# satoken/dafs

Hardware: AMD Instinct MI355X
Metric: seq-pairs/sec (all-pairs ProbCons pair-HMM posteriors + sparse rows + sim) (higher is better)
Workload: dtype f32; 1 GPU; N=128 L~150 synthetic random RNA (seed 12345), 8128 pairs; align_model=ProbCons, kernel=k_pairhmm3<G=32,W=6> x 4064 waves

## Files before the change

dafs_amd/csrc/call_host.h:

```cpp
#pragma once
#include <errno.h>
#include <math.h>
#include <stddef.h>
#include <stdint.h>
#include <stdlib.h>
#include <vector>

#include "../../include/dafs_hip.h"
#include "last_error.h"
#include "mix64.h"

namespace dafs {

struct carve {
  size_t top = 0;
  size_t take(size_t bytes) { const size_t at = top; top += (bytes + 255) & ~(size_t)255; return at; }
  size_t bytes() const { return top; }
  size_t reserve_bytes() const { return top + 256; }
};

inline uint64_t env_uint(const char* name, uint64_t lo, uint64_t hi, uint64_t fallback) {
  const char* e = getenv(name);
  if (!e || *e < '0' || *e > '9') return fallback;
  char* end = nullptr;
  errno = 0;
  const unsigned long long v = strtoull(e, &end, 10);
  return *end || errno == ERANGE || v < lo || v > hi ? fallback : (uint64_t)v;
}
inline bool env_off(const char* name) { return env_uint(name, 0, 0, 1) == 0; }
inline double env_double(const char* name, double fallback) {
  if (const char* e = getenv(name)) {
    char* end = nullptr;
    const double v = strtod(e, &end);
    if (end != e && v >= 0.0) return v;
  }
  return fallback;
}

inline int refuse(const char* what) {
  set_last_error(what);
  return DAFS_HIP_EINVAL;
}

inline bool structure_ok(const uint32_t* ss, uint32_t L, std::vector<uint8_t>& used) {
  used.assign(L, 0);
  for (uint32_t col = 0; col < L; ++col) {
    const uint32_t p = ss[col];
    if (p == DAFS_HIP_NONE) continue;
    if (p <= col || p >= L || used[col] || used[p]) return false;
    used[col] = used[p] = 1;
  }
  return true;
}

inline double nj_pair_distance(int model, uint32_t mism, uint32_t comp) {
  const double kQ = 1048576.0, kCapK = 3.0 * 1048576.0;
  if (model == DAFS_NJ_P) return comp ? (double)mism / (double)comp : 1.0;
  if (comp == 0 || 4 * (uint64_t)mism >= 3 * (uint64_t)comp) return 3.0;
  const double x = 1.0 - (4.0 * (double)mism) / (3.0 * (double)comp);
  double k = floor(-0.75 * log(x) * kQ + 0.5);
  if (!(k < kCapK)) k = kCapK;
  return k / kQ;
}

}
```

dafs_amd/csrc/pair_sweeps.h:

```cpp
#pragma once
#include <hip/hip_runtime.h>
#include <stdint.h>
#include <stdlib.h>
#include "../../include/dafs_hip.h"
#include "hip_util.h"

namespace dafs {

__device__ __forceinline__ int dpp_row_shr1(int fill, int v) { return __builtin_amdgcn_update_dpp(fill, v, 0x111, 0xF, 0xF, false); }
__device__ __forceinline__ int dpp_row_shl1(int fill, int v) { return __builtin_amdgcn_update_dpp(fill, v, 0x101, 0xF, 0xF, false); }
__device__ __forceinline__ int dpp_wave_shr1(int fill, int v) { return __builtin_amdgcn_update_dpp(fill, v, 0x138, 0xF, 0xF, false); }
__device__ __forceinline__ int dpp_wave_shl1(int fill, int v) { return __builtin_amdgcn_update_dpp(fill, v, 0x130, 0xF, 0xF, false); }

template <int G>
__device__ __forceinline__ int shift_up1(int v, int fill, int t) {
  if constexpr (G == 16) return dpp_row_shr1(fill, v);
  const int r = dpp_wave_shr1(fill, v);
  if constexpr (G == 64) return r;
  return t == 0 ? fill : r;
}
template <int G>
__device__ __forceinline__ float shift_up1(float v, float fill, int t) {
  return __int_as_float(shift_up1<G>(__float_as_int(v), __float_as_int(fill), t));
}
template <int G>
__device__ __forceinline__ int shift_down1(int v, int fill, int t) {
  if constexpr (G == 16) return dpp_row_shl1(fill, v);
  const int r = dpp_wave_shl1(fill, v);
  if constexpr (G == 64) return r;
  return t == G - 1 ? fill : r;
}
template <int G>
__device__ __forceinline__ float shift_down1(float v, float fill, int t) {
  return __int_as_float(shift_down1<G>(__float_as_int(v), __float_as_int(fill), t));
}

template <int G, int W>
__device__ __forceinline__ int pair_width(int L2) {
  if constexpr (W == 1) return 1;
  int m = L2;
#pragma unroll
  for (int o = G; o < 64; o <<= 1) m = max(m, __shfl_xor(m, o));
  m = __builtin_amdgcn_readfirstlane(m);
  return (m + 1 <= G * (W - 1)) ? W - 1 : W;
}

template <int WR>
struct pair_rec {
  static constexpr int Q = (2 + WR + 3) / 4;
  static constexpr int D = 4 * Q;
};
template <int G, int W, int WR, bool dense, bool staged, class Args, class Post>
__device__ __forceinline__ bool pair_finish(const Args& a, float* __restrict__ slab, float* __restrict__ list, int list_cap, uint32_t* __restrict__ s_rowptr,
                                            uint2* __restrict__ stage, int E, int lane, int t, int g, int L1, int L2, int nsteps, bool act, uint32_t task,
                                            float th, Post post) {
  const int tlast = (L2 >= 0 ? L2 : 0) / WR;
  const int j0 = t * WR;
  typedef uint32_t u32x4 __attribute__((ext_vector_type(4)));
  const __amdgpu_buffer_rsrc_t list_rs = __builtin_amdgcn_make_buffer_rsrc((void*)list, 0, list_cap * 256, 0x00020000);
  constexpr uint32_t NO_RECORD = 0x80000000u;
  int colcnt[WR];
  float simv = 0.0f;
  uint32_t nnz = 0;
  int slab_nrec = 0;
  {
    float pdp[WR];
    int ptr[WR];
#pragma unroll
    for (int c = 0; c < WR; ++c) { pdp[c] = 0.0f; ptr[c] = 0; colcnt[c] = 0; }
    float lastdp = 0.0f, dgdp = 0.0f;
    int lasttr = 0, dgtr = 0, lastcnt = 0;
    uint32_t rowacc = 0;
    if (t == G - 1) s_rowptr[0] = 0;
    int nrec = 0;
    bool ovf = false;
    float sva[WR], svb[WR];
#pragma unroll
    for (int c = 0; c < WR; ++c) sva[c] = slab[c * 64 + lane];
#pragma unroll
    for (int c = 0; c < WR; ++c) svb[c] = slab[(W + c) * 64 + lane];
#pragma unroll
    for (int c = 0; c < WR; ++c) asm volatile("" : "+v"(sva[c]), "+v"(svb[c]));
    auto step = [&](const int s, float (&sv)[WR]) __attribute__((always_inline)) {
      const int i = s - t;
      const bool rowv = (i >= 0) && (i <= L1);
      float* __restrict__ slab_s = slab + (size_t)s * (W * 64);
      const float rdp = shift_up1<G>(lastdp, 0.0f, t);
      const int rtr = shift_up1<G>(lasttr, 0, t), rcnt = shift_up1<G>(lastcnt, 0, t);
      float ddp = dgdp, ldp = rdp;
      int dtr = dgtr, ltr = rtr, run = rcnt;
      float pp[WR];
      post(sv, pp);
      {
        const float* __restrict__ slab_n = slab + (size_t)min(s + 2, nsteps - 1) * (W * 64);
#pragma unroll
        for (int c = 0; c < WR; ++c) sv[c] = slab_n[c * 64 + lane];
      }
      uint32_t emask = 0;
#pragma unroll
      for (int c = 0; c < WR; ++c) {
        const int j = j0 + c;
        const bool v = rowv && (j <= L2);
        const bool inner = v && i >= 1 && j >= 1;
        const float p = pp[c];
        const bool entry = inner && (p >= th) && (p > th);
        if (dense) slab_s[c * 64 + lane] = entry ? p : 0.0f;
        const float udp = pdp[c];
        const int utr = ptr[c];
        const float dpe = entry ? ddp + p : -1.0f;
        const bool fl = dpe < ldp;
        float dp = fl ? ldp : dpe;
        int tr = fl ? ltr : dtr;
        const bool fu = dp < udp;
        dp = fu ? udp : dp;
        tr = (fu ? utr : tr) + 1;
        if (!inner) { dp = 0.0f; tr = 0; }
        ddp = udp; dtr = utr;
        pdp[c] = dp; ptr[c] = tr;
        ldp = dp; ltr = tr;
        const int e = entry ? 1 : 0;
        run += e;
        colcnt[c] += e;
        emask |= (uint32_t)e << c;
      }
      if (!dense) {
        const bool fits = (nrec + 1) * pair_rec<WR>::D <= list_cap;
        const bool app = emask != 0 && fits;
        ovf = ovf || (emask != 0 && !fits);
        float w[pair_rec<WR>::D];
        w[0] = __uint_as_float(emask);
        w[1] = __int_as_float((i - 1) | (rcnt << 16));
#pragma unroll
        for (int c = 0; c < WR; ++c) w[2 + c] = pp[c];
#pragma unroll
        for (int c = 2 + WR; c < pair_rec<WR>::D; ++c) w[c] = 0.0f;
        const uint32_t ro = app ? (uint32_t)(((uint32_t)nrec * pair_rec<WR>::Q * 64 + lane) * 16) : NO_RECORD;
#if !defined(PAIR_EXP_NORECSTORE)
#pragma unroll
        for (int q = 0; q < pair_rec<WR>::Q; ++q) {
          const u32x4 d = {__float_as_uint(w[4 * q]), __float_as_uint(w[4 * q + 1]), __float_as_uint(w[4 * q + 2]), __float_as_uint(w[4 * q + 3])};
          __builtin_amdgcn_raw_buffer_store_b128(d, list_rs, (int)(ro + q * 1024), 0, 0);
        }
#else
        (void)ro; (void)list_rs;
#endif
        nrec += app ? 1 : 0;
      }
      dgdp = rdp; dgtr = rtr;
      lastdp = ldp; lasttr = ltr; lastcnt = run;
      if (i == L1 && t == tlast) {
        const int cl = L2 - j0;
        float sdp = 0.0f;
        int str = 1;
#pragma unroll
        for (int c = 0; c < WR; ++c)
          if (c == cl) { sdp = pdp[c]; str = ptr[c]; }
        simv = sdp / (float)str;
      }
      if (t == G - 1 && rowv && i >= 1) {
        rowacc += (uint32_t)run;
        s_rowptr[i] = rowacc;
      }
    };
    const int nrun = dense ? nsteps : (nsteps + 1) & ~1;
    for (int s = 0; s < nrun; s += 2) {
      step(s, sva);
      if (dense && s + 1 >= nsteps) break;
      step(s + 1, svb);
    }
    nnz = rowacc;
    if (!dense && __any(ovf)) return false;
    slab_nrec = nrec;
  }
  nnz = __shfl(nnz, g * G + (G - 1));
  simv = __shfl(simv, g * G + tlast);

  int colbase[WR];
  {
    int mine = 0;
#pragma unroll
    for (int c = 0; c < WR; ++c) mine += colcnt[c];
    int incl = mine;
#pragma unroll
    for (int o = 1; o < G; o <<= 1) {
      const int up = __shfl_up(incl, o, G);
      if (t >= o) incl += up;
    }
    int run = incl - mine;
#pragma unroll
    for (int c = 0; c < WR; ++c) { colbase[c] = run; run += colcnt[c]; }
  }

#if defined(PAIR_EXP_STOP) && PAIR_EXP_STOP == 3
  if (simv != 12345.0f || nnz != 12345u || colbase[WR - 1] != 12345) return true;
#endif
  unsigned long long off = 0;
  if (t == 0 && act) off = atomicAdd(a.pool_top, 2ull * nnz);
  off = __shfl(off, g * G);
  const bool ok = act && (off + 2ull * nnz <= a.pool_cap);
  if (act && !ok && t == 0) atomicExch(a.status, DAFS_HIP_EOVERFLOW);
  const uint64_t rp = act ? a.rp_off[task] : 0;
  if (act && t == 0) {
    a.pair_off[task] = off;
    a.pair_nnz[task] = nnz;
    a.sim[task] = simv;
  }
  wave_lds_fence();
  if (act) {
    for (int r = t; r <= L1; r += G) a.rowptr_pool[rp + r] = s_rowptr[r];
    if (t == 0) a.rowptr_pool[rp + L1 + 1] = 0;
#pragma unroll
    for (int c = 0; c < WR; ++c) {
      const int j = j0 + c;
      if (j >= 1 && j <= L2) a.rowptr_pool[rp + L1 + 1 + j] = (uint32_t)(colbase[c] + colcnt[c]);
    }
  }

  if (!dense) {
// ... 285 lines not shown
```

dafs_amd/csrc/pairhmm3.hip:

```cpp
#include <hip/hip_runtime.h>
#include <stdint.h>
#include <stdlib.h>
#include "../../include/dafs_hip.h"
#include "pc_math.h"
#include "hip_util.h"
#include "stage.h"
#include "pair_sweeps.h"

namespace dafs {

template <int G, int W, int WR>
__device__ __forceinline__ void pairhmm3_pair(const dafs_pairhmm3_args& a, const pc_tables* tab, const float* s_match, const float* s_ins, const float2* s_mi,
                                              float* __restrict__ slab, float* __restrict__ list, int list_cap, uint32_t* __restrict__ s_rowptr, uint2* __restrict__ s_stage, int E, int lane, int t, int g,
                                              int L1, int L2, int nsteps, bool act, uint32_t task,
                                              const uint8_t* __restrict__ s1, const uint8_t* __restrict__ s2) {
  const float LZ = PC_LOG_ZERO_S;
  const float i0 = a.model.init[0], i1 = a.model.init[1], i2 = a.model.init[2];
  const float tMM = a.model.trans[0][0], tMX = a.model.trans[0][1], tMY = a.model.trans[0][2];
  const float tXM = a.model.trans[1][0], tXX = a.model.trans[1][1];
  const float tYM = a.model.trans[2][0], tYY = a.model.trans[2][2];
  const int j0 = t * WR;
  const int tlast = (L2 >= 0 ? L2 : 0) / WR;

  int cc[WR + 1];
#pragma unroll
  for (int c = 0; c <= WR; ++c) {
    const int j = j0 + c;
    cc[c] = (j >= 1 && j <= L2) ? (int)s2[j - 1] : 6;
  }
  const int c1first = act ? (int)s1[0] : 6;
  const int c2first = act ? (int)s2[0] : 6;
  const float fM11 = i0 + s_match[c1first * 8 + c2first];
  const float fX10 = i1 + s_ins[c1first];
  const float fY01 = i2 + s_ins[c2first];

  float endM = LZ, endX = LZ, endY = LZ;
  {
    float pM[WR], pX[WR], pY[WR];
#pragma unroll
    for (int c = 0; c < WR; ++c) pM[c] = pX[c] = pY[c] = LZ;
    float lastM = LZ, lastX = LZ, lastY = LZ;
    float dgM = LZ, dgX = LZ, dgY = LZ;
    int c1n = 6;
    for (int s = 0; s < nsteps; ++s) {
      const int i = s - t;
      float* __restrict__ slab_s = slab + (size_t)s * (W * 64);
      const int c1 = c1n;
      c1n = (i >= 0 && i < L1) ? (int)s1[i] : 6;
      const float rM = shift_up1<G>(lastM, LZ, t), rX = shift_up1<G>(lastX, LZ, t), rY = shift_up1<G>(lastY, LZ, t);
      const float insc1 = s_ins[c1];
      const float2* __restrict__ mi_row = s_mi + c1 * 8;
      float2 mi_prev = make_float2(0.0f, 0.0f), mi_prev2 = mi_prev;
      float m1prev = LZ, xpend = LZ;
#pragma unroll
      for (int it = 0; it < WR + 2; ++it) {
        float x[4], y[4], o[4];
#pragma unroll
        for (int n = 0; n < 4; ++n) x[n] = y[n] = LZ;
        if (it < WR) {
          const float dM = it == 0 ? dgM : pM[it > 0 ? it - 1 : 0], dX = it == 0 ? dgX : pX[it > 0 ? it - 1 : 0];
          x[0] = dM + tMM; y[0] = dX + tXM;
          x[1] = pM[it] + tMX; y[1] = pX[it] + tXX;
        }
        if (it >= 1 && it - 1 < WR) {
          const int c = it - 1;
          const float dY = c == 0 ? dgY : pY[c > 0 ? c - 1 : 0];
          x[2] = m1prev; y[2] = dY + tYM;
        }
        if (it >= 2) {
          const int c = it - 2;
          const float lM = c == 0 ? rM : pM[c > 0 ? c - 1 : 0], lY = c == 0 ? rY : pY[c > 0 ? c - 1 : 0];
          x[3] = lM + tMY; y[3] = lY + tYY;
        }
        float2 mi_now = make_float2(0.0f, 0.0f);
        if (it < WR) mi_now = mi_row[cc[it]];
        pc_log_add_n<4>(tab, x, y, o);
        if (it >= 1 && it - 1 < WR) {
          const int c = it - 1;
          float mv = o[2] + mi_prev.x;
          if (c <= 1 && s <= 2) {
            const int j = j0 + c;
            if (i <= 1 && j <= 1) mv = (i == 1 && j == 1) ? fM11 : LZ;
          }
          pM[c] = mv;
          pX[c] = xpend;
#if !defined(PAIR_EXP_NOSTORE)
          slab_s[c * 64 + lane] = mv;
#endif
        }
        if (it < WR) {
          m1prev = o[0];
          float xv = insc1 + o[1];
          if (it <= 1 && s <= 2) {
            const int j = j0 + it;
            if (i <= 1 && j <= 1) xv = (i == 1 && j == 0) ? fX10 : LZ;
          }
          xpend = xv;
        }
        if (it >= 2) {
          const int c = it - 2;
          float yv = mi_prev2.y + o[3];
          if (c <= 1 && s <= 2) {
            const int j = j0 + c;
            if (i <= 1 && j <= 1) yv = (i == 0 && j == 1) ? fY01 : LZ;
          }
          pY[c] = yv;
        }
        mi_prev2 = mi_prev;
        mi_prev = mi_now;
      }
      dgM = rM; dgX = rX; dgY = rY;
      lastM = pM[WR - 1]; lastX = pX[WR - 1]; lastY = pY[WR - 1];
      if (i == L1 && t == tlast) {
        const int cl = L2 - j0;
#pragma unroll
        for (int c = 0; c < WR; ++c)
          if (c == cl) { endM = pM[c]; endX = pX[c]; endY = pY[c]; }
      }
    }
  }
#if defined(PAIR_EXP_STOP) && PAIR_EXP_STOP == 1
  if (endM != 12345.0f) return;
#endif
  float totF = LZ;
  totF = pc_log_add_s(tab, totF, endM + i0);
  totF = pc_log_add_s(tab, totF, endX + i1);
  totF = pc_log_add_s(tab, totF, endY + i2);
  totF = __shfl(totF, g * G + tlast);

  float capM = LZ, capX = LZ, capY = LZ;
  {
    float pM[WR], pX[WR];
#pragma unroll
    for (int c = 0; c < WR; ++c) pM[c] = pX[c] = LZ;
    float firstM = LZ, firstY = LZ;
    float dgM = LZ;
    int c1raw;
    float fwd[WR];
    {
      const float* __restrict__ q = slab + (size_t)(nsteps - 1) * (W * 64);
#pragma unroll
      for (int c = 0; c < WR; ++c) fwd[c] = q[c * 64 + lane];
      c1raw = (int)s1[max(min(nsteps - 1 - t, L1 - 1), 0)];
#pragma unroll
      for (int c = 0; c < WR; ++c) asm volatile("" : "+v"(fwd[c]));
      asm volatile("" : "+v"(c1raw));
    }
    for (int s = 0; s < nsteps; ++s) {
      const int sf = nsteps - 1 - s;
      const int i = sf - t;
      float* __restrict__ slab_s = slab + (size_t)sf * (W * 64);
      const float* __restrict__ slab_p = slab + (size_t)(sf > 0 ? sf - 1 : 0) * (W * 64);
      const int c1 = (i >= 0 && i < L1) ? c1raw : 6;
      c1raw = (int)s1[max(min(i - 1, L1 - 1), 0)];
      const float rM = shift_down1<G>(firstM, LZ, t), rY = shift_down1<G>(firstY, LZ, t);
      const float insc1 = s_ins[c1];
      const float2* __restrict__ mi_row = s_mi + c1 * 8;
      float bm1prev = LZ, by0prev = LZ, yprev = LZ, insprev = 0.0f;
      float2 mi_next = mi_row[cc[WR]];
#pragma unroll
      for (int it = 0; it < WR + 1; ++it) {
        float x[4], y[4], o[4];
        float by0now = LZ, insnow = 0.0f;
#pragma unroll
        for (int n = 0; n < 4; ++n) x[n] = y[n] = LZ;
        if (it < WR) {
          const int c = WR - 1 - it;
          const int j = j0 + c;
          const float2 mi = mi_next;
          const float dM = c == WR - 1 ? dgM : pM[c < WR - 1 ? c + 1 : 0];
          const float pxy = dM + mi.x;
          float bm = pxy + tMM, bx = pxy + tXM, by = pxy + tYM;
          if (i == L1 && j == L2) { bm = i0; bx = i1; by = i2; }
          const float tx = pX[c] + insc1;
          x[0] = bm; y[0] = tx + tMX;
          x[1] = bx; y[1] = tx + tXX;
          by0now = by;
          insnow = mi.y;
          if (c >= 1) mi_next = mi_row[cc[c]];
        }
        if (it >= 1) {
          const int c = WR - it;
          const float rgY = c == WR - 1 ? rY : yprev;
          const float ty = rgY + insprev;
          x[2] = bm1prev; y[2] = ty + tMY;
          x[3] = by0prev; y[3] = ty + tYY;
        }
        pc_log_add_n<4>(tab, x, y, o);
        if (it >= 1) {
          const int c = WR - it;
          const int j = j0 + c;
          pM[c] = o[2];
          yprev = o[3];
          slab_s[c * 64 + lane] = fwd[c] + o[2];
          fwd[c] = slab_p[c * 64 + lane];
          if (c <= 1) {
            if (i == 1 && j == 1) capM = o[2];
            if (i == 1 && j == 0) capX = pX[c];
            if (i == 0 && j == 1) capY = o[3];
          }
        }
        if (it < WR) {
          const int c = WR - 1 - it;
          bm1prev = o[0];
          by0prev = by0now;
          insprev = insnow;
          pX[c] = o[1];
        }
      }
      dgM = rM;
      firstM = pM[0];
      firstY = yprev;
    }
  }
#if defined(PAIR_EXP_STOP) && PAIR_EXP_STOP == 2
  if (capM != 12345.0f) return;
#endif
  capM = __shfl(capM, g * G + (1 / WR));
  capX = __shfl(capX, g * G);
  capY = __shfl(capY, g * G + (1 / WR));
  float totB = fM11 + capM;
  totB = pc_log_add_s(tab, totB, fX10 + capX);
  totB = pc_log_add_s(tab, totB, fY01 + capY);
  const float total = (totF + totB) / 2;

  auto post = [total, tab](const float (&sv)[WR], float (&p)[WR]) {
    float e[WR];
#pragma unroll
    for (int c = 0; c < WR; ++c) {
      const float v = (sv[c] - total) * (1.0f / PC_SCALE);
      e[c] = v < 0.0f ? v : 0.0f;
    }
    pc_exp_n<WR>(tab, e, p);
  };
  if (a.th < 0.002f || !pair_finish<G, W, WR, false, true>(a, slab, list, list_cap, s_rowptr, s_stage, E, lane, t, g, L1, L2, nsteps, act, task, a.th, post))
    (void)pair_finish<G, W, WR, true, true>(a, slab, list, list_cap, s_rowptr, s_stage, E, lane, t, g, L1, L2, nsteps, act, task, a.th, post);
}

template <int G, int W, int OCC>
__global__ __launch_bounds__(256, OCC) void k_pairhmm3(dafs_pairhmm3_args a, uint32_t slab_steps, uint32_t rp_cap, uint32_t emit_e) {
  constexpr int NG = 64 / G;
  extern __shared__ __attribute__((aligned(16))) uint32_t s_dyn[];
  __shared__ float s_match[56];
  __shared__ float s_ins[8];
  __shared__ float2 s_mi[56];
  __shared__ pc_tables s_tab;
  pc_tables_init(&s_tab, threadIdx.x);
  if (threadIdx.x < 56) s_match[threadIdx.x] = (&a.model.match[0][0])[threadIdx.x];
  if (threadIdx.x < 8) s_ins[threadIdx.x] = a.model.ins[threadIdx.x];
  if (threadIdx.x < 56) s_mi[threadIdx.x] = make_float2((&a.model.match[0][0])[threadIdx.x], a.model.ins[threadIdx.x & 7]);
  __syncthreads();
  pc_tables_init2(&s_tab, threadIdx.x, blockDim.x);
  __syncthreads();

  const int lane = threadIdx.x & 63;
  const int t = lane % G;
  const int g = lane / G;
  const int wave_in_wg = threadIdx.x >> 6;
  const uint32_t wave = __builtin_amdgcn_readfirstlane(blockIdx.x * 4 + wave_in_wg);
  const size_t plane = (size_t)slab_steps * W * 64;
  float* __restrict__ slab = a.scratch + (size_t)wave * plane * 2;
  float* __restrict__ list = slab + plane;
  const int list_cap = (int)(slab_steps * W);
  uint32_t* __restrict__ s_rowptr = s_dyn + (size_t)(wave_in_wg * NG + g) * rp_cap;
  uint2* __restrict__ s_stage = (uint2*)(s_dyn + (size_t)4 * NG * rp_cap) + (size_t)(wave_in_wg * NG + g) * (emit_e + G);

  for (;;) {
    uint32_t base = 0;
    if (lane == 0) base = atomicAdd(a.queue, (uint32_t)NG);
    base = __builtin_amdgcn_readfirstlane(base);
    if (base >= a.ntasks) break;
    const uint32_t task = base + g;
    const bool act = task < a.ntasks;
    dafs_pair_task tk = {0, 0, 0, 0};
    if (act) tk = a.tasks[task];
    const int L1 = act ? (int)tk.len1 : -1;
    const int L2 = act ? (int)tk.len2 : -1;
    const uint8_t* __restrict__ s1 = a.codes + tk.off1;
    const uint8_t* __restrict__ s2 = a.codes + tk.off2;
    int maxL1 = L1;
#pragma unroll
    for (int o = G; o < 64; o <<= 1) maxL1 = max(maxL1, __shfl_xor(maxL1, o));
    const int nsteps = __builtin_amdgcn_readfirstlane(maxL1) + G;
    if (pair_width<G, W>(L2) == W)
      pairhmm3_pair<G, W, W>(a, &s_tab, s_match, s_ins, s_mi, slab, list, list_cap, s_rowptr, s_stage, (int)emit_e, lane, t, g, L1, L2, nsteps, act, task, s1, s2);
    else
      pairhmm3_pair<G, W, (W > 1 ? W - 1 : 1)>(a, &s_tab, s_match, s_ins, s_mi, slab, list, list_cap, s_rowptr, s_stage, (int)emit_e, lane, t, g, L1, L2, nsteps, act, task, s1, s2);
  }
}

#define V(G, W, OCC) {G, W, (const void*)k_pairhmm3<G, W, OCC>, 0, OCC}
#ifdef PAIR_ONLY_VARIANTS
static pair_variant k_variants[] = {PAIR_ONLY_VARIANTS};
#else
static pair_variant k_variants[] = {
    V(16, 2, 4), V(16, 3, 4), V(16, 4, 4), V(16, 5, 4), V(16, 6, 4), V(16, 7, 3), V(16, 8, 3), V(16, 10, 2), V(16, 11, 2), V(16, 12, 2), V(16, 14, 1), V(16, 16, 1),
    V(32, 2, 4), V(32, 3, 4), V(32, 4, 4), V(32, 5, 4), V(32, 6, 4), V(32, 7, 3), V(32, 8, 3), V(32, 10, 2), V(32, 12, 2), V(32, 14, 1), V(32, 16, 1),
    V(64, 1, 4), V(64, 2, 4), V(64, 3, 4), V(64, 4, 4), V(64, 5, 4), V(64, 6, 4), V(64, 7, 3), V(64, 8, 3), V(64, 10, 2), V(64, 12, 2), V(64, 14, 1), V(64, 16, 1), V(64, 24, 1), V(64, 32, 1),
};
#endif
#undef V
static const int k_nvariants = (int)(sizeof k_variants / sizeof k_variants[0]);

}

using namespace dafs;

extern "C" int dafs_hipk_pairhmm_plan(uint32_t ntasks, uint32_t max_len1, uint32_t max_len2, dafs_pairhmm_plan* plan) {
  if (!plan || ntasks == 0 || max_len1 == 0 || max_len2 == 0) return DAFS_HIP_EINVAL;
  return pair_choose(k_variants, k_nvariants, ntasks, max_len1, max_len2, 2, 600.0, 370.0, 0.83, 0.17, plan);
}

extern "C" int dafs_hipk_pairhmm3_launch(const dafs_pairhmm3_args* args, const dafs_pairhmm_plan* plan, void* hip_stream) {
  if (!args || !plan) return DAFS_HIP_EINVAL;
  if (args->ntasks == 0) return DAFS_HIP_OK;
  pair_variant* v = nullptr;
  for (pair_variant& c : k_variants)
    if (c.G == (int)plan->group && c.W == (int)plan->width) v = &c;
  if (!v || plan->nwaves % 4 || plan->nwaves == 0) return DAFS_HIP_EINVAL;
  const uint64_t per_wave = (uint64_t)plan->slab_steps * plan->width * 64 * sizeof(float) * 2;
  if (per_wave && plan->nwaves > plan->scratch_bytes / per_wave) return DAFS_HIP_EINVAL;
  const uint32_t rp_cap = plan->slab_steps - plan->group + 1;
  const size_t rp_lds = pair_rowptr_lds(v->G, rp_cap);
  if (rp_lds > kPairRowptrLdsMax) return DAFS_HIP_ETOOLONG;
  size_t lds = 0;
  uint32_t emit_e = pair_emit_window(*v, rp_lds, &lds);
  if (lds + (size_t)v->lds_static > 64 * 1024 && !lds_optin_once(v->fn, 160 * 1024 - v->lds_static, v->optin)) return DAFS_HIP_ELAUNCH;
  dafs_pairhmm3_args a = *args;
  {
    float* f = &a.model.init[0];
    for (size_t k = 0; k < sizeof a.model / sizeof(float); ++k) f[k] *= 32.0f;
  }
  uint32_t steps = plan->slab_steps, cap = rp_cap;
  void* params[] = {&a, &steps, &cap, &emit_e};
  hipError_t launch_err = hipSuccess;
  STAGE_LAUNCH(dafs::ST_PAIRHMM3, (hipStream_t)hip_stream) launch_err = hipLaunchKernel(v->fn, dim3(plan->nwaves / 4), dim3(256), params, lds, (hipStream_t)hip_stream);
  if (hip_check(launch_err)) return DAFS_HIP_ELAUNCH;
  return DAFS_HIP_OK;
}
```

include/dafs_hip.h:

```cpp
#ifndef DAFS_HIP_H
#define DAFS_HIP_H
#include <stddef.h>
#include <stdint.h>

#ifdef __cplusplus
extern "C" {
#endif

#define DAFS_HIP_NONE 0xFFFFFFFFu

enum {
  DAFS_HIP_OK = 0,
  DAFS_HIP_EINVAL = -1,
  DAFS_HIP_ENODEV = -2,
  DAFS_HIP_ENOMEM = -3,
  DAFS_HIP_ETOOLONG = -4,
  DAFS_HIP_EOVERFLOW = -5,
  DAFS_HIP_ELAUNCH = -6,
  DAFS_HIP_ECOMM = -7
};
const char* dafs_hip_strerror(int code);
const char* dafs_hip_last_error(void);

enum { DAFS_ALIGN_PROBCONS = 0, DAFS_ALIGN_CONTRALIGN = 1 };
enum { DAFS_FOLD_CONTRAFOLD = 0 };


typedef struct {
  uint32_t off1, len1;
  uint32_t off2, len2;
} dafs_pair_task;

typedef struct {
  uint32_t group;
  uint32_t width;
  uint32_t nwaves;
  uint32_t slab_steps;
  uint64_t scratch_bytes;
} dafs_pairhmm_plan;

typedef struct {
  float init[3];
  float trans[3][3];
  float match[7][8];
  float ins[8];
} dafs_pairhmm3_model;

typedef struct {
  const uint8_t* codes;
  const dafs_pair_task* tasks;
  uint32_t ntasks;
  float th;
  float* scratch;
  uint32_t* queue;
  const uint64_t* rp_off;
  uint32_t* rowptr_pool;
  uint32_t* ent_col;
  float* ent_val;
  unsigned long long* pool_top;
  uint64_t pool_cap;
  uint64_t* pair_off;
  uint32_t* pair_nnz;
  float* sim;
  int* status;
  dafs_pairhmm3_model model;
} dafs_pairhmm3_args;

int dafs_hipk_pairhmm_plan(uint32_t ntasks, uint32_t max_len1, uint32_t max_len2, dafs_pairhmm_plan* plan);
int dafs_hipk_pairhmm3_launch(const dafs_pairhmm3_args* args, const dafs_pairhmm_plan* plan, void* hip_stream);
void dafs_hip_pairhmm3_default_model(dafs_pairhmm3_model* m);
uint8_t dafs_hip_residue_code(char c);

typedef struct {
  float match[5][5];
  float insert[5];
  float single[5];
  float pair[5][5];
} dafs_pairhmm5_model;

typedef struct {
  const uint8_t* codes;
  const dafs_pair_task* tasks;
  uint32_t ntasks;
  float th;
  float* scratch;
  uint32_t* queue;
  const uint64_t* rp_off;
  uint32_t* rowptr_pool;
  uint32_t* ent_col;
  float* ent_val;
  unsigned long long* pool_top;
  uint64_t pool_cap;
  uint64_t* pair_off;
  uint32_t* pair_nnz;
  float* sim;
  int* status;
  dafs_pairhmm5_model model;
} dafs_pairhmm5_args;

int dafs_hipk_pairhmm5_plan(uint32_t ntasks, uint32_t max_len1, uint32_t max_len2, dafs_pairhmm_plan* plan);
int dafs_hipk_pairhmm5_launch(const dafs_pairhmm5_args* args, const dafs_pairhmm_plan* plan, void* hip_stream);
void dafs_hip_pairhmm5_default_model(dafs_pairhmm5_model* m);

typedef struct dafs_hip_ctx dafs_hip_ctx;
int dafs_hip_create(int device, dafs_hip_ctx** ctx);
void dafs_hip_destroy(dafs_hip_ctx* ctx);

int dafs_hip_set_sequences(dafs_hip_ctx* ctx, uint32_t nseq, const char* const* seqs, const uint32_t* lens);
int dafs_hip_set_families(dafs_hip_ctx* ctx, uint32_t nfam, const uint32_t* first);
int dafs_hip_align_posteriors(dafs_hip_ctx* ctx, int model, float th, uint64_t pair_begin, uint64_t pair_end);
int dafs_hip_align_result_size(dafs_hip_ctx* ctx, uint64_t* npairs, uint64_t* total_nnz, uint64_t* total_rowptr);
int dafs_hip_align_fetch(dafs_hip_ctx* ctx, uint32_t* pair_x, uint32_t* pair_y, float* sim, uint32_t* nnz,
                         uint32_t* rowptr, uint32_t* col, float* val);

int dafs_hip_mp_result_size(dafs_hip_ctx* ctx, int relaxed, uint64_t* npairs, uint64_t* total_nnz, uint64_t* total_rowptr);
int dafs_hip_mp_fetch(dafs_hip_ctx* ctx, int relaxed, uint32_t* pair_x, uint32_t* pair_y, uint32_t* nnz,
                      uint32_t* rowptr, uint32_t* col, float* val);
int dafs_hip_set_mp(dafs_hip_ctx* ctx, const uint32_t* nnz, const uint32_t* rowptr, const uint32_t* col, const float* val);
int dafs_hip_mp_install(dafs_hip_ctx* ctx, int relaxed, const uint32_t* nnz, const uint32_t* rowptr, const uint32_t* col,
                        const float* val, const float* sim);
int dafs_hip_get_sim(dafs_hip_ctx* ctx, float* sim);
int dafs_hip_similarity(dafs_hip_ctx* ctx, int model, float th, uint64_t max_bytes, uint64_t* n_ranges_out);
int dafs_host_similarity_ranges(uint32_t n, const uint32_t* lens, uint64_t max_bytes, uint64_t* end, uint64_t cap, uint64_t* n_ranges);

int dafs_hip_structure_scores(dafs_hip_ctx* ctx, uint64_t* T, uint64_t* terms, uint64_t* W);
float dafs_host_structure_score(uint64_t T, uint64_t Wx, uint64_t Wy);
float dafs_host_mix_score(float sim, float str, float w);
enum { DAFS_SCORE_SEQUENCE = 0, DAFS_SCORE_STRUCTURE = 1, DAFS_SCORE_MIX = 2 };
int dafs_hip_similarity_scored(dafs_hip_ctx* ctx, int model, float th, uint64_t max_bytes, int kind, float weight, uint64_t* n_ranges_out);
int dafs_hip_get_pair_scores(dafs_hip_ctx* ctx, float* seq, float* str);

int dafs_hip_set_bp(dafs_hip_ctx* ctx, const uint32_t* rowptr, const uint32_t* col, const float* val);
int dafs_hip_bp_result_size(dafs_hip_ctx* ctx, int relaxed, uint64_t* total_nnz, uint64_t* total_rowptr);
int dafs_hip_bp_fetch(dafs_hip_ctx* ctx, int relaxed, uint32_t* rowptr, uint32_t* col, float* val);

int dafs_hip_fold_posteriors(dafs_hip_ctx* ctx, int model, float th);
int dafs_hip_fold_posteriors_begin(dafs_hip_ctx* ctx, int model, float th);
int dafs_hip_fold_posteriors_end(dafs_hip_ctx* ctx);
int dafs_hip_fold_posteriors_constrained_begin(dafs_hip_ctx* ctx, int model, float th, const char* const* constraints);
int dafs_hip_fold_posteriors_constrained(dafs_hip_ctx* ctx, int model, float th, const char* const* constraints);
int dafs_hip_fold_posteriors_levels_begin(dafs_hip_ctx* ctx, int model, float th, uint32_t nlevels, const char* const* constraints);
int dafs_hip_fold_posteriors_levels(dafs_hip_ctx* ctx, int model, float th, uint32_t nlevels, const char* const* constraints);
int dafs_hip_fold_posterior_dense(dafs_hip_ctx* ctx, const char* seq, uint32_t len, const char* constraint, float* post,
                                  float* logz);

int dafs_host_build_tree(uint32_t n, const float* sim, float* score, int32_t* left, int32_t* right);
enum { DAFS_CLUSTER_THRESHOLD = 0, DAFS_CLUSTER_COUNT = 1 };
int dafs_host_cluster_cut(uint32_t n, const float* score, const int32_t* left, const int32_t* right, int mode, float threshold,
                          uint32_t count, uint32_t* labels, uint32_t* n_clusters);

enum { DAFS_LINKAGE_SINGLE = 1, DAFS_LINKAGE_COMPLETE = 2, DAFS_LINKAGE_AVERAGE = 3 };
int dafs_hip_linkage_tree(dafs_hip_ctx* ctx, int linkage, uint32_t n, const float* sim, float* score, int32_t* left, int32_t* right);
size_t dafs_hipk_linkage_workspace(uint32_t n);
int dafs_hipk_linkage(int linkage, uint32_t n, const float* d_sim, void* d_workspace, float* d_score, int32_t* d_left, int32_t* d_right,
                      void* hip_stream);

int dafs_hip_nj_tree(dafs_hip_ctx* ctx, uint32_t n, const double* dist, int32_t* left, int32_t* right, double* length);
size_t dafs_hipk_nj_workspace(uint32_t n);
int dafs_hipk_nj(uint32_t n, const double* d_dist, void* d_workspace, int32_t* d_left, int32_t* d_right, double* d_length,
                 void* hip_stream);
enum { DAFS_NJ_P = 0, DAFS_NJ_JC = 1 };
int dafs_host_nj_distances(uint32_t n, const uint32_t* ident, const uint32_t* aligned, int model, double* dist);
int dafs_host_newick(uint32_t n, const char* const* names, const int32_t* left, const int32_t* right, const double* length, char** out);
enum {
  DAFS_PHYLOGENY_NO_PAIRWISE = 0,
  DAFS_PHYLOGENY_NO_SEED_EACH,
  DAFS_PHYLOGENY_TOO_MANY_ROWS,
  DAFS_PHYLOGENY_MODEL_NEEDS_TREE,
  DAFS_PHYLOGENY_UNKNOWN_MODEL,
  DAFS_PHYLOGENY_COV_TREE_NEEDS_NULL,
  DAFS_PHYLOGENY_UNKNOWN_COV_TREE
};
const char* dafs_host_phylogeny_refusal(int which);
enum {
  DAFS_BOOTSTRAP_NEEDS_TREE = 0,
  DAFS_BOOTSTRAP_COUNT,
  DAFS_BOOTSTRAP_NEEDS_REPLICATES,
  DAFS_BOOTSTRAP_NO_COLUMN
};
const char* dafs_host_bootstrap_refusal(int which);

int dafs_hip_nj_trees(dafs_hip_ctx* ctx, uint32_t n, uint32_t count, const double* dist, int32_t* left, int32_t* right, double* length);
size_t dafs_hipk_nj_batch_workspace(uint32_t n, uint32_t count);
int dafs_hipk_nj_batch(uint32_t n, uint32_t count, const double* d_dist, void* d_workspace, int32_t* d_left, int32_t* d_right,
                       double* d_length, void* hip_stream);
int dafs_hip_alignment_bootstrap(dafs_hip_ctx* ctx, uint32_t n, uint32_t len, const uint8_t* cell, const uint8_t* use, int model, uint32_t B,
                                 uint64_t seed, const int32_t* main_left, const int32_t* main_right, int32_t* support, int32_t* rep_left,
                                 int32_t* rep_right);
int dafs_hip_bootstrap_alignment(dafs_hip_ctx* ctx, uint32_t n, uint32_t len, const uint8_t* cell, const uint8_t* use, uint64_t seed, uint32_t k,
                                 uint8_t* out_cell);
uint64_t dafs_hip_bootstrap_fixups(void);
int dafs_host_tree_support(uint32_t n, const int32_t* left, const int32_t* right, uint32_t B, const int32_t* rep_left,
                           const int32_t* rep_right, int32_t* support);
int dafs_host_newick_support(uint32_t n, const char* const* names, const int32_t* left, const int32_t* right, const double* length,
                             const int32_t* support, uint32_t B, char** out);
int dafs_host_support_table(uint32_t n, const char* const* names, const int32_t* left, const int32_t* right, const int32_t* support,
                            uint32_t B, uint64_t seed, int model, char** out);

int dafs_host_merge_added(uint32_t C, uint32_t k, const uint32_t* lens, const uint32_t* z, uint32_t* seed_col, uint32_t* res_col,
                          uint32_t* width);

void dafs_host_free(void* text);
char dafs_host_pp_char(double p);
int dafs_host_stockholm_names(uint32_t n, const char* const* headers, char** names);
int dafs_host_stockholm_block(const char* tree_line, uint32_t n, uint32_t len, const char* const* names, const char* const* rows,
                              const double* const* residue_rel, const double* col_rel, const char* ss, const uint8_t* rf,
                              const char* cov, char** block);
int dafs_host_stockholm_block_rows(const char* tree_line, uint32_t n, uint32_t len, const char* const* names, const char* const* rows,
                                   const double* const* residue_rel, const double* col_rel, const char* ss, const uint8_t* rf,
                                   const char* cov, const char* const* row_ss, char** block);
int dafs_host_stockholm_block_merged(uint32_t n, uint32_t len, const char* const* names, const char* const* rows,
                                     const double* const* residue_rel, const char* ss, const uint8_t* rf, double* col_rel, char** block);
const char* dafs_host_merged_refusal(void);
uint8_t dafs_host_cov_code(char residue);
int dafs_host_cov_ss_cons(uint32_t len, const uint32_t* ss, const double* pair_e, double e_max, char** chars);
int dafs_host_covariation_table(uint32_t n, uint32_t len, const uint8_t* code, const uint32_t* ss, const uint32_t* best,
                                const double* best_score, const double* best_e, const double* pair_score, const double* pair_e,
                                const uint32_t* pair_rows, const uint32_t* pair_canonical, const uint32_t* pair_types, char** table);
int dafs_host_pairwise_table(uint64_t npairs, const uint32_t* x, const uint32_t* y, uint32_t nnames, const char* const* names,
                             const double* sim, const double* score, const int64_t* iterations, char** table);
int dafs_host_cluster_table(uint32_t n, const char* const* headers, const uint32_t* length, const uint32_t* labels, const float* score,
                            const int32_t* left, const int32_t* right, const float* sim, char** table);
// ... 240 lines not shown
```

Measured before the change: 6.230 million seq-pairs/s.

## Prefilter posterior candidates during backward pass using forward-backward log-sum cut

During the backward sweep, each cell's forward+backward log sum is compared against a host-precomputed conservative log-domain cut derived from the threshold. Only rows with candidate cells are written as compact records into the list buffer instead of writing the full slab. The finish stage then exponentiates just those candidates and replays the sparse DP from them. A trust check on forward/backward total agreement, plus overflow detection, falls back to the classic full-slab path. This aims to cut slab stores and the exp work on the full matrix, at the cost of extra code, a second backward pass on fallback, and a reliance on the cut bound being conservative.

```diff
diff --git a/dafs_amd/csrc/call_host.h b/dafs_amd/csrc/call_host.h
--- a/dafs_amd/csrc/call_host.h
+++ b/dafs_amd/csrc/call_host.h
@@ -53,6 +53,41 @@
   return true;
 }
 
+inline float pair_cut(float th) {
+  static const std::vector<double> M = [] {
+    static const double e[5][5] = {
+        {0.01973899026052090000, 0.13822379685007000000, 0.48056651562365000000, 0.99326940370383500000, 0.99906756856399500000},
+        {0.00940528203591384000, 0.09414963667859410000, 0.40825793595877300000, 0.93933625499130400000, 0.98369508190545300000},
+        {0.00217245711583303000, 0.03484829428350620000, 0.22118199801337800000, 0.67049462206469500000, 0.83556950223398500000},
+        {0.00012398771025456900, 0.00349155785951272000, 0.03727721426017900000, 0.17974997741536900000, 0.33249299994217400000},
+        {0.00000051741713416603, 0.00002721456879608080, 0.00053418601865636800, 0.00464101989351936000, 0.01507447981459420000}};
+    const int n = (16 * 1024) - 512;
+    std::vector<double> m((size_t)n + 1, 0.0);
+    const double h = 1.0 / 1024.0;
+    for (int k = 1; k <= n; ++k) {
+      const double a = -16.0 + (k - 1) * h, b = -16.0 + k * h;
+      const double* q = e[b <= -8.0 ? 4 : b <= -4.0 ? 3 : b <= -2.0 ? 2 : b <= -1.0 ? 1 : 0];
+      const double pa = (((q[0] * a + q[1]) * a + q[2]) * a + q[3]) * a + q[4];
+      const double pb = (((q[0] * b + q[1]) * b + q[2]) * b + q[3]) * b + q[4];
+      const double x = -a;
+      const double d2 = 12.0 * q[0] * x * x + 6.0 * q[1] * x + 2.0 * q[2];
+      const double d1 = q[3] - 2.0 * q[2] * x - 4.0 * q[0] * x * x * x;
+      const double bound = (d1 > 0.0 ? pb : (pa > pb ? pa : pb) + d2 * h * h / 8.0) + 1e-12;
+      m[(size_t)k] = bound > m[(size_t)k - 1] ? bound : m[(size_t)k - 1];
+    }
+    return m;
+  }();
+  size_t lo = 0, hi = M.size() - 1;
+  if (!(M[hi] <= (double)th)) {
+    while (hi - lo > 1) {
+      const size_t mid = (lo + hi) / 2;
+      if (M[mid] <= (double)th) lo = mid; else hi = mid;
+    }
+    hi = lo;
+  }
+  return (float)(-16.0 + (double)hi / 1024.0);
+}
+
 inline double nj_pair_distance(int model, uint32_t mism, uint32_t comp) {
   const double kQ = 1048576.0, kCapK = 3.0 * 1048576.0;
   if (model == DAFS_NJ_P) return comp ? (double)mism / (double)comp : 1.0;
diff --git a/dafs_amd/csrc/pair_sweeps.h b/dafs_amd/csrc/pair_sweeps.h
--- a/dafs_amd/csrc/pair_sweeps.h
+++ b/dafs_amd/csrc/pair_sweeps.h
@@ -50,10 +50,11 @@
   static constexpr int Q = (2 + WR + 3) / 4;
   static constexpr int D = 4 * Q;
 };
-template <int G, int W, int WR, bool dense, bool staged, class Args, class Post>
+template <int G, int W, int WR, bool dense, bool staged, bool picked = false, class Args, class Post>
 __device__ __forceinline__ bool pair_finish(const Args& a, float* __restrict__ slab, float* __restrict__ list, int list_cap, uint32_t* __restrict__ s_rowptr,
                                             uint2* __restrict__ stage, int E, int lane, int t, int g, int L1, int L2, int nsteps, bool act, uint32_t task,
-                                            float th, Post post) {
+                                            float th, Post post, int ncand = 0) {
+  static_assert(!(picked && dense), "the candidate form is a sparse form");
   const int tlast = (L2 >= 0 ? L2 : 0) / WR;
   const int j0 = t * WR;
   typedef uint32_t u32x4 __attribute__((ext_vector_type(4)));
@@ -63,7 +64,137 @@
   float simv = 0.0f;
   uint32_t nnz = 0;
   int slab_nrec = 0;
-  {
+  if constexpr (picked) {
+    constexpr int Q = pair_rec<WR>::Q;
+    const __amdgpu_buffer_rsrc_t cand_rs = __builtin_amdgcn_make_buffer_rsrc((void*)slab, 0, list_cap * 256, 0x00020000);
+    auto rec_off = [lane](const int k, const bool have) { return have ? (uint32_t)(((uint32_t)k * Q * 64 + lane) * 16) : NO_RECORD; };
+    {
+      int maxc = ncand;
+#pragma unroll
+      for (int o = 1; o < 64; o <<= 1) maxc = max(maxc, __shfl_xor(maxc, o));
+      maxc = __builtin_amdgcn_readfirstlane(maxc);
+      constexpr int K = 2;
+      for (int k0 = 0; k0 < maxc; k0 += K) {
+        u32x4 r[K][Q];
+#pragma unroll
+        for (int kk = 0; kk < K; ++kk)
+#pragma unroll
+          for (int q = 0; q < Q; ++q) r[kk][q] = __builtin_amdgcn_raw_buffer_load_b128(cand_rs, (int)(rec_off(k0 + kk, k0 + kk < ncand) + q * 1024), 0, 0);
+#pragma unroll
+        for (int kk = 0; kk < K; ++kk) {
+          uint32_t w[4 * Q];
+#pragma unroll
+          for (int q = 0; q < Q; ++q) { w[4 * q] = r[kk][q].x; w[4 * q + 1] = r[kk][q].y; w[4 * q + 2] = r[kk][q].z; w[4 * q + 3] = r[kk][q].w; }
+          float sv[WR], pp[WR];
+#pragma unroll
+          for (int c = 0; c < WR; ++c) sv[c] = __uint_as_float(w[2 + c]);
+          post(sv, pp);
+          uint32_t exact = 0;
+#pragma unroll
+          for (int c = 0; c < WR; ++c) exact |= (uint32_t)((pp[c] >= th) && (pp[c] > th) ? 1 : 0) << c;
+          w[0] &= exact;
+#pragma unroll
+          for (int c = 0; c < WR; ++c) w[2 + c] = __float_as_uint(pp[c]);
+#pragma unroll
+          for (int q = 0; q < Q; ++q) {
+            const u32x4 d = {w[4 * q], w[4 * q + 1], w[4 * q + 2], w[4 * q + 3]};
+            __builtin_amdgcn_raw_buffer_store_b128(d, cand_rs, (int)(rec_off(k0 + kk, k0 + kk < ncand) + q * 1024), 0, 0);
+          }
+        }
+      }
+    }
+#if defined(PAIR_EXP_STOP) && PAIR_EXP_STOP == 4
+    if (ncand != 12345) return true;
+#endif
+    float pdp[WR];
+    int ptr[WR];
+#pragma unroll
+    for (int c = 0; c < WR; ++c) { pdp[c] = 0.0f; ptr[c] = 0; colcnt[c] = 0; }
+    float lastdp = 0.0f, dgdp = 0.0f;
+    int lasttr = 0, dgtr = 0, lastcnt = 0;
+    uint32_t rowacc = 0;
+    if (t == G - 1) s_rowptr[0] = 0;
+    int nrec = 0;
+    int left = ncand;
+    u32x4 cur[Q], pend[Q];
+#pragma unroll
+    for (int q = 0; q < Q; ++q) cur[q] = __builtin_amdgcn_raw_buffer_load_b128(cand_rs, (int)(rec_off(left - 1, left > 0) + q * 1024), 0, 0);
+#pragma unroll
+    for (int q = 0; q < Q; ++q) { asm volatile("" : "+v"(cur[q])); pend[q] = cur[q]; }
+    bool took = false;
+    for (int s = 0; s < nsteps; ++s) {
+      const int i = s - t;
+      const bool rowv = (i >= 0) && (i <= L1);
+      if (took) {
+#pragma unroll
+        for (int q = 0; q < Q; ++q) cur[q] = pend[q];
+      }
+      const bool hit = left > 0 && (int)cur[0].y == i;
+      left -= hit ? 1 : 0;
+#pragma unroll
+      for (int q = 0; q < Q; ++q) pend[q] = __builtin_amdgcn_raw_buffer_load_b128(cand_rs, (int)(rec_off(left - 1, hit && left > 0) + q * 1024), 0, 0);
+      took = hit;
+      uint32_t w[4 * Q];
+#pragma unroll
+      for (int q = 0; q < Q; ++q) { w[4 * q] = cur[q].x; w[4 * q + 1] = cur[q].y; w[4 * q + 2] = cur[q].z; w[4 * q + 3] = cur[q].w; }
+      const uint32_t emask = hit ? w[0] : 0u;
+      const float rdp = shift_up1<G>(lastdp, 0.0f, t);
+      const int rtr = shift_up1<G>(lasttr, 0, t), rcnt = shift_up1<G>(lastcnt, 0, t);
+      float ddp = dgdp, ldp = rdp;
+      int dtr = dgtr, ltr = rtr, run = rcnt;
+#pragma unroll
+      for (int c = 0; c < WR; ++c) {
+        const int j = j0 + c;
+        const bool inner = rowv && (j <= L2) && i >= 1 && j >= 1;
+        const bool entry = ((emask >> c) & 1u) != 0;
+        const float p = __uint_as_float(w[2 + c]);
+        const float udp = pdp[c];
+        const int utr = ptr[c];
+        const float dpe = entry ? ddp + p : -1.0f;
+        const bool fl = dpe < ldp;
+        float dp = fl ? ldp : dpe;
+        int tr = fl ? ltr : dtr;
+        const bool fu = dp < udp;
+        dp = fu ? udp : dp;
+        tr = (fu ? utr : tr) + 1;
+        if (!inner) { dp = 0.0f; tr = 0; }
+        ddp = udp; dtr = utr;
+        pdp[c] = dp; ptr[c] = tr;
+        ldp = dp; ltr = tr;
+        const int e = entry ? 1 : 0;
+        run += e;
+        colcnt[c] += e;
+      }
+      {
+        w[0] = emask;
+        w[1] = (uint32_t)((i - 1) | (rcnt << 16));
+        const uint32_t ro = emask != 0 ? (uint32_t)(((uint32_t)nrec * Q * 64 + lane) * 16) : NO_RECORD;
+#pragma unroll
+        for (int q = 0; q < Q; ++q) {
+          const u32x4 d = {w[4 * q], w[4 * q + 1], w[4 * q + 2], w[4 * q + 3]};
+          __builtin_amdgcn_raw_buffer_store_b128(d, list_rs, (int)(ro + q * 1024), 0, 0);
+        }
+        nrec += emask != 0 ? 1 : 0;
+      }
+      dgdp = rdp; dgtr = rtr;
+      lastdp = ldp; lasttr = ltr; lastcnt = run;
+      if (i == L1 && t == tlast) {
+        const int cl = L2 - j0;
+        float sdp = 0.0f;
+        int str = 1;
+#pragma unroll
+        for (int c = 0; c < WR; ++c)
+          if (c == cl) { sdp = pdp[c]; str = ptr[c]; }
+        simv = sdp / (float)str;
+      }
+      if (t == G - 1 && rowv && i >= 1) {
+        rowacc += (uint32_t)run;
+        s_rowptr[i] = rowacc;
+      }
+    }
+    nnz = rowacc;
+    slab_nrec = nrec;
+  } else {
     float pdp[WR];
     int ptr[WR];
 #pragma unroll
diff --git a/dafs_amd/csrc/pairhmm3.hip b/dafs_amd/csrc/pairhmm3.hip
--- a/dafs_amd/csrc/pairhmm3.hip
+++ b/dafs_amd/csrc/pairhmm3.hip
@@ -1,7 +1,9 @@
 #include <hip/hip_runtime.h>
 #include <stdint.h>
 #include <stdlib.h>
+#include <type_traits>
 #include "../../include/dafs_hip.h"
+#include "call_host.h"
 #include "pc_math.h"
 #include "hip_util.h"
 #include "stage.h"
@@ -9,8 +11,14 @@
 
 namespace dafs {
 
+struct pair_pick {
+  float cut;
+  float trust;
+  uint32_t on;
+};
+
 template <int G, int W, int WR>
-__device__ __forceinline__ void pairhmm3_pair(const dafs_pairhmm3_args& a, const pc_tables* tab, const float* s_match, const float* s_ins, const float2* s_mi,
+__device__ __forceinline__ void pairhmm3_pair(const dafs_pairhmm3_args& a, const pair_pick& pk, const pc_tables* tab, const float* s_match, const float* s_ins, const float2* s_mi,
                                               float* __restrict__ slab, float* __restrict__ list, int list_cap, uint32_t* __restrict__ s_rowptr, uint2* __restrict__ s_stage, int E, int lane, int t, int g,
                                               int L1, int L2, int nsteps, bool act, uint32_t task,
                                               const uint8_t* __restrict__ s1, const uint8_t* __restrict__ s2) {
@@ -129,7 +137,14 @@
   totF = __shfl(totF, g * G + tlast);
 
   float capM = LZ, capX = LZ, capY = LZ;
-  {
+  int ncand = 0;
+  auto backward = [&](auto pick_tag) __attribute__((always_inline)) -> bool {
+    constexpr bool pick = decltype(pick_tag)::value;
+    typedef uint32_t u32x4 __attribute__((ext_vector_type(4)));
+    const __amdgpu_buffer_rsrc_t cand_rs = __builtin_amdgcn_make_buffer_rsrc((void*)list, 0, list_cap * 256, 0x00020000);
+    bool ovf = false;
+    capM = capX = capY = LZ;
+    ncand = 0;
     float pM[WR], pX[WR];
 #pragma unroll
     for (int c = 0; c < WR; ++c) pM[c] = pX[c] = LZ;
@@ -158,6 +173,8 @@
       const float2* __restrict__ mi_row = s_mi + c1 * 8;
       float bm1prev = LZ, by0prev = LZ, yprev = LZ, insprev = 0.0f;
       float2 mi_next = mi_row[cc[WR]];
+      float sums[WR];
+      uint32_t cmask = 0;
 #pragma unroll
       for (int it = 0; it < WR + 1; ++it) {
         float x[4], y[4], o[4];
@@ -192,7 +209,13 @@
           const int j = j0 + c;
           pM[c] = o[2];
           yprev = o[3];
-          slab_s[c * 64 + lane] = fwd[c] + o[2];
+          const float sum = fwd[c] + o[2];
+          if constexpr (pick) {
+            sums[c] = sum;
+            cmask |= (uint32_t)(sum - totF >= pk.cut ? 1 : 0) << c;
+          } else {
+            slab_s[c * 64 + lane] = sum;
+          }
           fwd[c] = slab_p[c * 64 + lane];
           if (c <= 1) {
             if (i == 1 && j == 1) capM = o[2];
@@ -208,21 +231,62 @@
           pX[c] = o[1];
         }
       }
+      if constexpr (pick) {
+        constexpr int Q = pair_rec<WR>::Q, D = pair_rec<WR>::D;
+        const bool fits = (ncand + 1) * D <= list_cap;
+        const bool app = cmask != 0 && fits;
+        ovf = ovf || (cmask != 0 && !fits);
+        uint32_t w[D];
+        w[0] = cmask;
+        w[1] = (uint32_t)i;
+#pragma unroll
+        for (int c = 0; c < WR; ++c) w[2 + c] = __float_as_uint(sums[c]);
+#pragma unroll
+        for (int c = 2 + WR; c < D; ++c) w[c] = 0u;
+        const uint32_t ro = app ? (uint32_t)(((uint32_t)ncand * Q * 64 + lane) * 16) : 0x80000000u;
+#pragma unroll
+        for (int q = 0; q < Q; ++q) {
+          const u32x4 d = {w[4 * q], w[4 * q + 1], w[4 * q + 2], w[4 * q + 3]};
+          __builtin_amdgcn_raw_buffer_store_b128(d, cand_rs, (int)(ro + q * 1024), 0, 0);
+        }
+        ncand += app ? 1 : 0;
+      }
       dgM = rM;
       firstM = pM[0];
       firstY = yprev;
     }
-  }
+    return ovf;
+  };
+  float totB = LZ, total = LZ;
+  auto totals = [&]() __attribute__((always_inline)) {
+    capM = __shfl(capM, g * G + (1 / WR));
+    capX = __shfl(capX, g * G);
+    capY = __shfl(capY, g * G + (1 / WR));
+    totB = fM11 + capM;
+    totB = pc_log_add_s(tab, totB, fX10 + capX);
+    totB = pc_log_add_s(tab, totB, fY01 + capY);
+    total = (totF + totB) / 2;
+  };
+  bool picked = false;
+  if (pk.on && a.th >= 0.002f) {
+    const bool ovf = backward(std::true_type());
 #if defined(PAIR_EXP_STOP) && PAIR_EXP_STOP == 2
-  if (capM != 12345.0f) return;
-#endif
-  capM = __shfl(capM, g * G + (1 / WR));
-  capX = __shfl(capX, g * G);
-  capY = __shfl(capY, g * G + (1 / WR));
-  float totB = fM11 + capM;
-  totB = pc_log_add_s(tab, totB, fX10 + capX);
-  totB = pc_log_add_s(tab, totB, fY01 + capY);
-  const float total = (totF + totB) / 2;
+    if (capM != 12345.0f) return;
+#endif
+    totals();
+    const bool bad = act && (ovf || !(fabsf(totB - totF) <= pk.trust));
+    picked = !__any(bad);
+#if defined(PAIR_EXP_COUNT_CLASSIC)
+    if (!picked && act && t == 0) atomicAdd(a.status, 256);
+#endif
+  }
+  if (!picked) {
+    (void)backward(std::false_type());
+#if defined(PAIR_EXP_STOP) && PAIR_EXP_STOP == 2
+    if (capM != 12345.0f) return;
+#endif
+    totals();
+  }
 
   auto post = [total, tab](const float (&sv)[WR], float (&p)[WR]) {
     float e[WR];
@@ -233,12 +297,14 @@
     }
     pc_exp_n<WR>(tab, e, p);
   };
-  if (a.th < 0.002f || !pair_finish<G, W, WR, false, true>(a, slab, list, list_cap, s_rowptr, s_stage, E, lane, t, g, L1, L2, nsteps, act, task, a.th, post))
+  if (picked)
+    (void)pair_finish<G, W, WR, false, true, true>(a, list, slab, list_cap, s_rowptr, s_stage, E, lane, t, g, L1, L2, nsteps, act, task, a.th, post, ncand);
+  else if (a.th < 0.002f || !pair_finish<G, W, WR, false, true>(a, slab, list, list_cap, s_rowptr, s_stage, E, lane, t, g, L1, L2, nsteps, act, task, a.th, post))
     (void)pair_finish<G, W, WR, true, true>(a, slab, list, list_cap, s_rowptr, s_stage, E, lane, t, g, L1, L2, nsteps, act, task, a.th, post);
 }
 
 template <int G, int W, int OCC>
-__global__ __launch_bounds__(256, OCC) void k_pairhmm3(dafs_pairhmm3_args a, uint32_t slab_steps, uint32_t rp_cap, uint32_t emit_e) {
+__global__ __launch_bounds__(256, OCC) void k_pairhmm3(dafs_pairhmm3_args a, uint32_t slab_steps, uint32_t rp_cap, uint32_t emit_e, pair_pick pk) {
   constexpr int NG = 64 / G;
   extern __shared__ __attribute__((aligned(16))) uint32_t s_dyn[];
   __shared__ float s_match[56];
@@ -283,9 +349,9 @@
     for (int o = G; o < 64; o <<= 1) maxL1 = max(maxL1, __shfl_xor(maxL1, o));
     const int nsteps = __builtin_amdgcn_readfirstlane(maxL1) + G;
     if (pair_width<G, W>(L2) == W)
-      pairhmm3_pair<G, W, W>(a, &s_tab, s_match, s_ins, s_mi, slab, list, list_cap, s_rowptr, s_stage, (int)emit_e, lane, t, g, L1, L2, nsteps, act, task, s1, s2);
+      pairhmm3_pair<G, W, W>(a, pk, &s_tab, s_match, s_ins, s_mi, slab, list, list_cap, s_rowptr, s_stage, (int)emit_e, lane, t, g, L1, L2, nsteps, act, task, s1, s2);
     else
-      pairhmm3_pair<G, W, (W > 1 ? W - 1 : 1)>(a, &s_tab, s_match, s_ins, s_mi, slab, list, list_cap, s_rowptr, s_stage, (int)emit_e, lane, t, g, L1, L2, nsteps, act, task, s1, s2);
+      pairhmm3_pair<G, W, (W > 1 ? W - 1 : 1)>(a, pk, &s_tab, s_match, s_ins, s_mi, slab, list, list_cap, s_rowptr, s_stage, (int)emit_e, lane, t, g, L1, L2, nsteps, act, task, s1, s2);
   }
 }
 
@@ -310,6 +376,8 @@
   if (!plan || ntasks == 0 || max_len1 == 0 || max_len2 == 0) return DAFS_HIP_EINVAL;
   return pair_choose(k_variants, k_nvariants, ntasks, max_len1, max_len2, 2, 600.0, 370.0, 0.83, 0.17, plan);
 }
+
+extern "C" float dafs_hip_pair_cut(float th) { return pair_cut(th); }
 
 extern "C" int dafs_hipk_pairhmm3_launch(const dafs_pairhmm3_args* args, const dafs_pairhmm_plan* plan, void* hip_stream) {
   if (!args || !plan) return DAFS_HIP_EINVAL;
@@ -331,8 +399,11 @@
     float* f = &a.model.init[0];
     for (size_t k = 0; k < sizeof a.model / sizeof(float); ++k) f[k] *= 32.0f;
   }
+  const uint64_t margin = env_uint("DAFS_HIP_PAIR_PICK_MARGIN", 0, 8192, 128);
+  const float delta = (float)margin / 1024.0f;
+  pair_pick pk = {32.0f * (pair_cut(a.th) - delta), margin ? 32.0f * delta : -1.0f, env_off("DAFS_HIP_PAIR_PICK") ? 0u : 1u};
   uint32_t steps = plan->slab_steps, cap = rp_cap;
-  void* params[] = {&a, &steps, &cap, &emit_e};
+  void* params[] = {&a, &steps, &cap, &emit_e, &pk};
   hipError_t launch_err = hipSuccess;
   STAGE_LAUNCH(dafs::ST_PAIRHMM3, (hipStream_t)hip_stream) launch_err = hipLaunchKernel(v->fn, dim3(plan->nwaves / 4), dim3(256), params, lds, (hipStream_t)hip_stream);
   if (hip_check(launch_err)) return DAFS_HIP_ELAUNCH;
diff --git a/include/dafs_hip.h b/include/dafs_hip.h
--- a/include/dafs_hip.h
+++ b/include/dafs_hip.h
@@ -68,6 +68,7 @@
 
 int dafs_hipk_pairhmm_plan(uint32_t ntasks, uint32_t max_len1, uint32_t max_len2, dafs_pairhmm_plan* plan);
 int dafs_hipk_pairhmm3_launch(const dafs_pairhmm3_args* args, const dafs_pairhmm_plan* plan, void* hip_stream);
+float dafs_hip_pair_cut(float th);
 void dafs_hip_pairhmm3_default_model(dafs_pairhmm3_model* m);
 uint8_t dafs_hip_residue_code(char c);
 
```

New measurement: 6.997 million seq-pairs/s, median of 6. 1.12x the previous value.
